# IBM/AdaMML

Hardware: AMD Instinct MI355X
Metric: clips/sec (train fwd+bwd) RGB+Audio AdaMML @224^2, 5 seg (higher is better)
Workload: dtype bf16

## Files before the change

### adamml_amd/csrc/conv_gemm.hip

```cpp
#include "common.h"
#include "tile.h"
#include "conv_internal.h"
#include "../../include/adamml_hip.h"
#include <stdlib.h>
#include <stdio.h>


namespace {

constexpr int BP = 128;
constexpr int BK = 32;

struct ConvP {
    const bf16_t* x;
    const bf16_t* w;
    const float* in_scale;
    const float* in_shift;
    bf16_t* y;
    double* stats;
    int N, H, W, Cin, OH, OW, Cout, KH, KW, stride, pad, up, up_shift, act, accumulate;
    int P, K, cin_shift, n_ptiles, n_ctiles, tpb;
    size_t gx, gy;
    int in_gstride;
    const bf16_t* bn_z;
// ... 1201 lines not shown

extern "C" int adamml_conv_fwd_bn_add_next_supported(const adamml_conv_desc_t* d, int next_cout) {
    return d && next_cout > 0 && adamml_conv_fwd_bn_add_supported(d) && adamml_conv1x1_fadd_next_supported(d, next_cout) ? 1 : 0;
}

extern "C" int adamml_conv_fwd_bn_add_next(const adamml_conv_desc_t* d, const void* x, const void* w_packed, const float* in_scale,
                                           const float* in_shift, const float* bn_vec, const void* idn, const float* id_scale,
                                           const float* id_shift, int id_gstride, int act, void* out, uint8_t* mask_out, const void* w_next,
                                           void* y_next, double* stats_next, hipStream_t stream) {
    if (!d || !x || !w_packed || !bn_vec || !out || !w_next || !y_next) return adamml_set_error(ADAMML_EINVAL, "conv_fwd_bn_add_next: null argument");
    if (!adamml_conv_fwd_bn_add_next_supported(d, 64))
        return adamml_set_error(ADAMML_EUNSUPPORTED, "conv_fwd_bn_add_next: 1x1 / stride-1, 64 -> 256 channels, next conv 256 -> 64 only");
    return adamml_conv1x1_fadd_next_launch(d, x, w_packed, in_scale, in_shift, bn_vec, idn, id_scale, id_shift, id_gstride, act, out, mask_out,
                                           w_next, y_next, stats_next, stream);
}

extern "C" int adamml_conv_fwd_bn_add_tpool_supported(const adamml_conv_desc_t* d, int frames, int act, int lazy_input) {
    if (!adamml_conv_fwd_bn_add_supported(d)) return 0;
    if (!(frames == 2 || frames == 4 || frames == 8) || d->N % frames || d->Cout % 128 || act != ADAMML_ACT_RELU) return 0;
    if (lazy_input && d->Cin > 512) return 0;
    return 1;
}

extern "C" int adamml_conv_fwd_bn_add_tpool_streams(const adamml_conv_desc_t* d, int frames) {
    if (!d) return 0;
    if (adamml_conv1x1_fadd_tpool_stream_supported(d, frames)) return 2;
    return adamml_conv1x1_fadd_tpool_supported(d, frames) ? 1 : 0;
}

extern "C" int adamml_conv_fwd_bn_add_tpool(const adamml_conv_desc_t* d, const void* x, const void* w_packed, const float* in_scale,
                                            const float* in_shift, const float* bn_vec, const void* idn, const float* id_scale,
                                            const float* id_shift, int id_gstride, int act, int frames, void* pooled, uint16_t* code,
                                            hipStream_t stream) {
    if (!adamml_conv_fwd_bn_add_tpool_supported(d, frames, act, in_scale != nullptr))
        return adamml_set_error(ADAMML_EUNSUPPORTED, "conv_fwd_bn_add_tpool: 1x1 / stride-1 conv, Cout %% 128 == 0, ReLU, 2 / 4 / 8 frames per clip");
    if (!bn_vec || !idn || !pooled) return adamml_set_error(ADAMML_EINVAL, "conv_fwd_bn_add_tpool: null argument");
    if (adamml_conv1x1_fadd_tpool_stream_supported(d, frames))
        return adamml_conv1x1_fadd_tpool_stream_launch(d, x, w_packed, in_scale, in_shift, bn_vec, idn, id_scale, id_shift, id_gstride, act, frames, pooled,
                                                       code, stream);
    if (adamml_conv1x1_fadd_tpool_supported(d, frames))
        return adamml_conv1x1_fadd_tpool_launch(d, x, w_packed, in_scale, in_shift, bn_vec, idn, id_scale, id_shift, id_gstride, act, frames, pooled, code,
                                                stream);
    FaddEpi f{bn_vec, idn, id_scale, id_shift, id_gstride, act, nullptr, frames, pooled, code};
    return conv_launch(d, x, w_packed, in_scale, in_shift, pooled, nullptr, nullptr, nullptr, 0, stream, nullptr, nullptr, nullptr, nullptr, &f);
}

static int conv_dgrad_stride2(const adamml_conv_desc_t* d, const void* dz, const void* w, void* dx, int accumulate, double* sums,
                              const void* z_in, const float* bn_vec, int act, hipStream_t stream) {
    const adamml_conv_desc_t g = dgrad_desc(d, accumulate);
    const int taps = d->KH * d->KW;
    for (int ph = 0; ph < 2; ++ph)
        for (int pw = 0; pw < 2; ++pw) {
            DgradClass c;
            c.nt = 0; c.code = 0; c.ph = ph; c.pw = pw;
            c.OHc = (d->H - ph + 1) / 2; c.OWc = (d->W - pw + 1) / 2;
            if (c.OHc <= 0 || c.OWc <= 0) continue;
            for (int kh = 0; kh < d->KH; ++kh) {
                if ((ph + d->pad - kh) & 1) continue;
                const int dh = (ph + d->pad - kh) / 2;
                for (int kw = 0; kw < d->KW; ++kw) {
                    if ((pw + d->pad - kw) & 1) continue;
                    const int dw = (pw + d->pad - kw) / 2;
                    const unsigned wt = (unsigned)(taps - 1 - (kh * d->KW + kw));
                    c.code |= ((unsigned)dh | ((unsigned)dw << 1) | (wt << 2)) << (8 * c.nt);
                    ++c.nt;
                }
            }
            if (c.nt == 0 && accumulate) continue;
            int rc = conv_launch(&g, dz, w, nullptr, nullptr, dx, sums, z_in, bn_vec, act, stream, &c);
            if (rc) return rc;
        }
    return ADAMML_OK;
}

static bool dgrad_stride2_ok(const adamml_conv_desc_t* d) {
    const bool k3 = d->KH == 3 && d->KW == 3 && d->pad == 1, k1 = d->KH == 1 && d->KW == 1 && d->pad == 0;
    return d->stride == 2 && (k3 || k1) && (d->up <= 1) && ilog2_exact(d->Cout) >= 0 &&
           d->OH == (d->H + 2 * d->pad - d->KH) / 2 + 1 && d->OW == (d->W + 2 * d->pad - d->KW) / 2 + 1;
}

extern "C" int adamml_conv_bwd_data_bn(const adamml_conv_desc_t* d, const void* dz, const void* w_dgrad_packed, void* dx,
                                       const void* z_in, const float* bn_vec, int act, double* sums, hipStream_t stream) {
    if (!d || !z_in || !bn_vec || !sums) return adamml_set_error(ADAMML_EINVAL, "conv_bwd_data_bn: null argument");
    if (dgrad_stride2_ok(d)) return conv_dgrad_stride2(d, dz, w_dgrad_packed, dx, 0, sums, z_in, bn_vec, act, stream);
    const adamml_conv_desc_t g = dgrad_desc(d, 0, true);
    return conv_launch(&g, dz, w_dgrad_packed, nullptr, nullptr, dx, sums, z_in, bn_vec, act, stream);
}

extern "C" int adamml_conv_bwd_data_dual_supported(const adamml_conv_desc_t* d) {
    return d && d->KH == 1 && d->KW == 1 && d->stride == 1 && d->pad == 0 && d->Cout <= 512 && d->Cin % 8 == 0 && d->Cout % 8 == 0 ? 1 : 0;
}

extern "C" int adamml_conv_bwd_data_dual(const adamml_conv_desc_t* d, const void* g, const void* z, const float* aff, void* dz_side,
                                         const void* w_dgrad_packed, void* dx, int accumulate, const void* z_in, const float* bn_vec,
                                         int act, double* sums, hipStream_t stream) {
    if (!d || !g || !z || !aff) return adamml_set_error(ADAMML_EINVAL, "conv_bwd_data_dual: null argument");
    if (!adamml_conv_bwd_data_dual_supported(d))
        return adamml_set_error(ADAMML_EUNSUPPORTED, "conv_bwd_data_dual: only 1x1 / stride-1 convs with Cout <= 512");
    if ((z_in != nullptr) != (bn_vec != nullptr) || (z_in != nullptr) != (sums != nullptr))
        return adamml_set_error(ADAMML_EINVAL, "conv_bwd_data_dual: incomplete BatchNorm epilogue operands");
    if (z_in && accumulate) return adamml_set_error(ADAMML_EUNSUPPORTED, "conv_bwd_data_dual: the BatchNorm epilogue does not accumulate");
    if (adamml_conv1x1_narrow_dual_supported(d))
        return adamml_conv1x1_narrow_dual_launch(d, g, z, aff, dz_side, w_dgrad_packed, dx, accumulate, z_in, bn_vec, act, sums, stream);
    const adamml_conv_desc_t gd = dgrad_desc(d, accumulate);
    DualIn di{z, aff, dz_side};
    return conv_launch(&gd, g, w_dgrad_packed, nullptr, nullptr, dx, sums, z_in, bn_vec, act, stream, nullptr, nullptr, &di);
}

extern "C" int adamml_conv_bwd_data_alg_streams(const adamml_conv_desc_t* d) {
    return d && d->KH == 1 && d->KW == 1 && d->stride == 1 && d->pad == 0 && adamml_alg_stream_supported(d->Cout, d->Cin) ? 1 : 0;
}

extern "C" int adamml_conv_bwd_data_alg(const adamml_conv_desc_t* d, const void* g, const void* a, const float* a_scale, const float* a_shift,
                                        const void* w_alg, const float* epi_add, void* dx, int accumulate, const void* z_in,
                                        const float* bn_vec, int act, double* sums, hipStream_t stream) {
    if (!d || !g || !a || !w_alg || !epi_add || !dx) return adamml_set_error(ADAMML_EINVAL, "conv_bwd_data_alg: null argument");
    if (!(d->KH == 1 && d->KW == 1 && d->stride == 1 && d->pad == 0)) return adamml_set_error(ADAMML_EUNSUPPORTED, "conv_bwd_data_alg: only 1x1 / stride-1 convs");
    if ((z_in != nullptr) != (bn_vec != nullptr) || (z_in != nullptr) != (sums != nullptr))
        return adamml_set_error(ADAMML_EINVAL, "conv_bwd_data_alg: incomplete BatchNorm epilogue operands");
    if (z_in && accumulate) return adamml_set_error(ADAMML_EUNSUPPORTED, "conv_bwd_data_alg: the BatchNorm epilogue does not accumulate");
    if (adamml_alg_stream_supported(d->Cout, d->Cin))
        return adamml_alg_stream_launch(d, g, a, a_scale, a_shift, w_alg, epi_add, dx, accumulate, z_in, bn_vec, act, sums, stream);
    adamml_conv_desc_t gd = dgrad_desc(d, accumulate);
    gd.act = d->act; gd.in_gstride = d->in_gstride;
    CatIn c{a, d->Cin, (size_t)d->Cin * (d->Cout + d->Cin), epi_add};
    return conv_launch(&gd, g, w_alg, a_scale, a_shift, dx, sums, z_in, bn_vec, act, stream, nullptr, nullptr, nullptr, &c);
}

static bool res_1x1(const adamml_conv_desc_t* d) {
    return d && d->KH == 1 && d->KW == 1 && d->stride == 1 && d->pad == 0 && d->Cin % 8 == 0 && d->Cout % 8 == 0;
}

static bool res_3x3(const adamml_conv_desc_t* d) {
    return d && d->KH == 3 && d->KW == 3 && d->stride == 1 && d->pad == 1 && d->up <= 1 && d->Cin == d->Cout && d->Cin >= 64 &&
           ilog2_exact(d->Cin) >= 0 && d->OH == d->H && d->OW == d->W;
}

extern "C" int adamml_conv_bwd_data_res_supported(const adamml_conv_desc_t* d) {
    return res_1x1(d) || res_3x3(d) ? 1 : 0;
}

static bool res_3x3_c64(const adamml_conv_desc_t* d) {
    if (!res_3x3(d)) return false;
    const adamml_conv_desc_t g = dgrad_desc(d, 0, true);
    return adamml_conv3x3_c64_res_supported(&g);
}

extern "C" int adamml_conv_bwd_data_res_streams(const adamml_conv_desc_t* d) {
    if (res_3x3_c64(d)) return 2;
    return res_1x1(d) && adamml_res_stream_supported(d) ? 1 : 0;
}

extern "C" int adamml_conv_bwd_data_res(const adamml_conv_desc_t* d, const void* dz, const void* w_dgrad_packed, void* dx,
                                        int accumulate, const void* res_out, const uint8_t* res_mask, int res_act, const void* z_a, const float* vec_a,
                                        double* sums_a, const void* z_b, const float* vec_b, double* sums_b,
                                        hipStream_t stream) {
    if (!d || !res_out || !sums_a || (z_a && !vec_a)) return adamml_set_error(ADAMML_EINVAL, "conv_bwd_data_res: null argument");
    if ((z_b != nullptr) != (vec_b != nullptr) || (z_b != nullptr) != (sums_b != nullptr))
        return adamml_set_error(ADAMML_EINVAL, "conv_bwd_data_res: incomplete second BatchNorm operand");
    if (!adamml_conv_bwd_data_res_supported(d))
        return adamml_set_error(ADAMML_EUNSUPPORTED, "conv_bwd_data_res: only 1x1 / stride-1 convs and 3x3 / pad-1 / stride-1 convs with Cin == Cout (a power of two >= 64)");
    if (accumulate && res_mask && !z_a && res_1x1(d) && adamml_res_stream_supported(d))
        return adamml_res_stream_launch(d, dz, w_dgrad_packed, dx, res_mask, sums_a, z_b, vec_b, sums_b, stream);
    const adamml_conv_desc_t g = dgrad_desc(d, accumulate, d->KH > 1);
    if (!z_b && res_3x3_c64(d))
        return adamml_conv3x3_c64_res_launch(&g, dz, w_dgrad_packed, dx, res_out, res_mask, res_act, z_a, vec_a, sums_a, stream);
    ResEpi r{res_out, res_mask, res_act, z_b, vec_b, sums_b};
    return conv_launch(&g, dz, w_dgrad_packed, nullptr, nullptr, dx, sums_a, z_a, vec_a, ACT_NONE, stream, nullptr, &r);
}
// ... 45 lines not shown
```

### adamml_amd/csrc/conv_internal.h

```cpp
#pragma once
#include "common.h"
#include "../../include/adamml_hip.h"

void launch_wgrad_reduce(const float* ws, float* dw, size_t n, int nsplit, int taps, int cin, int store, int groups, hipStream_t stream);
int adamml_launch_split_reduce(const float* ws, float* dw, size_t n, int nsplit, hipStream_t stream, int taps = 1, int cin = 1);
int adamml_launch_split_reduce_grouped(const float* ws, float* out, size_t n, int nsplit, int groups, int cin, hipStream_t stream);

bool adamml_conv3x3_c64_supported(const adamml_conv_desc_t* d);
int adamml_conv3x3_c64_launch(const adamml_conv_desc_t* d, const void* x, const void* w_packed, const float* in_scale,
                              const float* in_shift, void* y, double* stats, const void* bn_z, const float* bn_vec, int bn_act,
                              hipStream_t stream);
bool adamml_conv3x3_c64_res_supported(const adamml_conv_desc_t* d);
int adamml_conv3x3_c64_res_launch(const adamml_conv_desc_t* d, const void* dz, const void* w_dgrad_packed, void* dx, const void* res_out,
                                  const uint8_t* res_mask, int res_act, const void* z_a, const float* vec_a, double* sums_a, hipStream_t stream);
bool adamml_conv3x3_c64_wgrad_supported(const adamml_conv_desc_t* d, int cin_true);
int adamml_conv3x3_c64_wgrad_blocks(const adamml_conv_desc_t* d, int* tpb_out);
int adamml_conv3x3_c64_wgrad_launch(const adamml_conv_desc_t* d, const void* dz, const void* x, const float* in_scale,
                                    const float* in_shift, float* ws, hipStream_t stream);

bool adamml_conv1x1_narrow_fwd_supported(const adamml_conv_desc_t* d);
int adamml_conv1x1_narrow_fwd_launch(const adamml_conv_desc_t* d, const void* x, const void* w_packed, const float* in_scale, const float* in_shift,
                                     void* y, double* stats, hipStream_t stream);
bool adamml_conv1x1_narrow_wgrad_supported(const adamml_conv_desc_t* d, int cin_true);
int adamml_conv1x1_narrow_wgrad_launch(const adamml_conv_desc_t* d, const void* dz, const void* x, const float* in_scale, const float* in_shift,
                                       float* ws, int max_blocks_per_group, int* nblk_out, hipStream_t stream);
bool adamml_conv1x1_narrow_dual_supported(const adamml_conv_desc_t* d);
int adamml_conv1x1_narrow_dual_launch(const adamml_conv_desc_t* d, const void* g, const void* z, const float* aff, void* dz_side,
                                      const void* w_dgrad_packed, void* dx, int accumulate, const void* z_in, const float* bn_vec, int act,
                                      double* sums, hipStream_t stream);
bool adamml_conv1x1_narrow_dgrad_epi_supported(const adamml_conv_desc_t* d);
int adamml_conv1x1_narrow_dgrad_epi_launch(const adamml_conv_desc_t* d, const void* dz, const void* w_packed, void* dx, const void* z_in,
                                           const float* bn_vec, int act, double* sums, hipStream_t stream);

bool adamml_conv1x1_wide_expand_supported(const adamml_conv_desc_t* d);
int adamml_conv1x1_wide_expand_launch(const adamml_conv_desc_t* d, const void* x, const void* w_packed, const float* in_scale, const float* in_shift,
                                      void* y, double* stats, hipStream_t stream);

int adamml_conv1x1_fadd_stream_supported(const adamml_conv_desc_t* d);
int adamml_conv1x1_fadd_stream_launch(const adamml_conv_desc_t* d, const void* x, const void* w_packed, const float* in_scale, const float* in_shift,
                                      const float* bn_vec, const void* idn, const float* id_scale, const float* id_shift, int id_gstride, int act,
                                      void* out, uint8_t* mask_out, hipStream_t stream);
int adamml_conv1x1_fadd_tpool_stream_supported(const adamml_conv_desc_t* d, int frames);
int adamml_conv1x1_fadd_tpool_stream_launch(const adamml_conv_desc_t* d, const void* x, const void* w_packed, const float* in_scale, const float* in_shift,
                                            const float* bn_vec, const void* idn, const float* id_scale, const float* id_shift, int id_gstride, int act,
                                            int frames, void* pooled, uint16_t* code, hipStream_t stream);

bool adamml_conv1x1_fadd_next_supported(const adamml_conv_desc_t* d, int next_cout);
int adamml_conv1x1_fadd_next_launch(const adamml_conv_desc_t* d, const void* x, const void* w_packed, const float* in_scale, const float* in_shift,
                                    const float* bn_vec, const void* idn, const float* id_scale, const float* id_shift, int id_gstride, int act,
                                    void* out, uint8_t* mask_out, const void* w1_packed, void* y1, double* stats1, hipStream_t stream);
bool adamml_conv1x1_fadd_tpool_supported(const adamml_conv_desc_t* d, int frames);
int adamml_conv1x1_fadd_tpool_launch(const adamml_conv_desc_t* d, const void* x, const void* w_packed, const float* in_scale, const float* in_shift,
                                     const float* bn_vec, const void* idn, const float* id_scale, const float* id_shift, int id_gstride, int act,
                                     int frames, void* pooled, uint16_t* code, hipStream_t stream);

bool adamml_alg_stream_supported(int Cout, int Cin);
int adamml_alg_stream_launch(const adamml_conv_desc_t* d, const void* g, const void* a, const float* a_scale, const float* a_shift,
                             const void* w_alg, const float* epi_add, void* dx, int accumulate, const void* z_in, const float* bn_vec,
                             int act, double* sums, hipStream_t stream);

int adamml_res_stream_supported(const adamml_conv_desc_t* d);
int adamml_res_stream_launch(const adamml_conv_desc_t* d, const void* dz, const void* w_dgrad_packed, void* dx, const uint8_t* res_mask, double* sums_a,
                             const void* z_b, const float* vec_b, double* sums_b, hipStream_t stream);
int adamml_res_prod_stream_supported(const adamml_conv_desc_t* d, int a_channels);
size_t adamml_res_prod_stream_workspace(const adamml_conv_desc_t* d);
int adamml_res_prod_stream_launch(const adamml_conv_desc_t* d, const void* dz, const void* w_dgrad_packed, void* dx, const uint8_t* res_mask,
                                  double* sums_a, const void* a, const float* a_scale, const float* a_shift, int a_act, int a_gstride,
                                  float* prod, void* workspace, size_t workspace_bytes, hipStream_t stream);
```

### adamml_amd/hip.py

```python
import ctypes
import os
from ctypes import c_void_p, c_int, c_int32, c_int64, c_float, c_double, c_size_t, c_char_p, POINTER, Structure, byref

import torch

_HERE = os.path.dirname(os.path.abspath(__file__))
LIB_PATH = os.environ.get("ADAMML_HIP_LIB") or os.path.join(_HERE, "libadamml_hip.so")

ACT_NONE, ACT_RELU, ACT_RELU6 = 0, 1, 2
STAT_SLOTS = 32


class ConvDesc(Structure):
    _fields_ = [(n, c_int32) for n in ("N", "H", "W", "Cin", "OH", "OW", "Cout", "KH", "KW", "stride", "pad", "up", "act",
                                      "accumulate", "groups", "in_gstride")]

    def __init__(self, *args, **kw):
        super().__init__(*args, **kw)
        if self.groups < 1:
            self.groups = 1


_P, _I, _F, _D, _Z, _L = c_void_p, c_int, c_float, c_double, c_size_t, c_int64
_DESC = POINTER(ConvDesc)
# ... 40 lines not shown
    "adamml_bn_eval_affine": [_P, _P, _P, _P, _F, _P, _P, _I, _P],
    "adamml_bn_act_add": [_P, _P, _P, _I, _I, _P, _P, _P, _I, _P, _Z, _I, _I, _P],
    "adamml_act_bwd_from_output": [_P, _P, _I, _P, _Z, _P],
    "adamml_bn_bwd_reduce": [_P, _P, _P, _I, _P, _Z, _I, _I, _P],
    "adamml_bn_bwd_finalize": [_P, _I, _I, _D, _P, _P, _P, _P, _P, _I, _F, _P],
    "adamml_bn_bwd_finalize_affine": [_P, _I, _I, _D, _P, _P, _P, _P, _P, _P, _I, _F, _P],
    "adamml_bn_bwd_apply": [_P, _P, _P, _I, _P, _P, _Z, _I, _I, _P],
    "adamml_maxpool2d_fwd": [_P, _P, _P, _I, _I, _P, _P, _P, _I, _I, _I, _I, _I, _I, _I, _P],
    "adamml_maxpool2d_bwd": [_P, _P, _P, _I, _I, _I, _I, _I, _I, _I, _P],
    "adamml_maxpool2d_bwd_bn_reduce": [_P, _P, _P, _P, _I, _P, _I, _I, _I, _I, _I, _I, _I, _P],
    "adamml_maxpool2d_bwd_bn_apply": [_P, _P, _P, _P, _I, _P, _P, _I, _I, _I, _I, _I, _I, _I, _P],
    "adamml_temporal_pool_fwd": [_P, _P, _P, _I, _I, _P, _I, _I, _Z, _I, _I, _I, _P],
    "adamml_temporal_pool_bwd": [_P, _P, _P, _P, _I, _I, _P, _I, _I, _Z, _I, _I, _I, _P],
    "adamml_temporal_pool_bwd_res": [_P, _P, _I, _P, _P, _P, _P, _I, _I, _I, _I, _I, _P],
    "adamml_gap_fwd": [_P, _P, _P, _I, _I, _P, _I, _I, _I, _I, _P],
    "adamml_gap_bwd": [_P, _P, _I, _I, _I, _P],
    "adamml_head_fwd": [_P, _P, _P, _I, _I, _P, _F, _P, _P, _P, _P, _I, _I, _I, _I, _I, _I, _P],
    "adamml_head_bwd": [_P, _P, _F, _P, _P, _P, _I, _I, _I, _I, _I, _P],
    "adamml_colsum_f32": [_P, _P, _I, _I, _I, _P],
    "adamml_clip_to_nhwc": [_P, _P, _I, _I, _I, _I, _I, _I, _I, _I, _I, _I, _P],
    "adamml_clip_u8_to_nhwc": [_P, _P, _I, _I, _I, _I, _I, _I, _I, _I, _I, _I, _P, _P, _I, _I, _P],
    "adamml_clip_u8_rgbdiff_to_nhwc": [_P, _P, _I, _I, _I, _I, _I, _I, _I, _I, _I, _I, _P, _P, _I, _P],
    "adamml_log_spectrogram": [_P, _P, _P, _I, _I, _I, _I, _I, _F, _P],
    "adamml_video_resample_u8": [_P, _L, _P, _I, _P, _I, _I, _I, _I, _I, _I, _P],
    "adamml_jpeg_decode_u8": [_P, _L, _P, _I, _P, _L, _P, _P, _L, _I, _P],
    "adamml_gemm_f32": [_P, _L, _L, _P, _L, _L, _P, _L, _L, _P, _I, _I, _I, _I, _I, _P],
    "adamml_sgd_step": [_P, _P, _P, _Z, _F, _F, _F, _I, _I, _P],
    "adamml_adam_step": [_P, _P, _P, _P, _Z, _F, _F, _F, _F, _F, _I, _P],
    "adamml_policy_head_fwd": [_P, _P, _I, _P, _P, _P, _P, _P, _F, _P, _P, _P, _P, _P, _P, _P, _I, _I, _I, _I, _P],
    "adamml_policy_head_bwd": [_P, _P, _P, _I, _P, _P, _F, _P, _P, _P, _P, _P, _I, _I, _I, _I, _P],
    "adamml_gumbel_gate_fwd": [_P, _P, _F, _P, _P, _I, _P],
    "adamml_gumbel_gate_bwd": [_P, _P, _F, _P, _I, _P],
    "adamml_fusion_fwd": [_P, _P, _P, _P, _I, _I, _I, _I, _P],
    "adamml_fusion_bwd": [_P, _P, _P, _P, _P, _P, _P, _I, _I, _I, _I, _P],
}

_lib = None


def load():
    global _lib
    if _lib is not None:
        return _lib
    if not os.path.exists(LIB_PATH):
        raise RuntimeError("adamml_amd: %s not found -- build it with `python -c 'import __graft_entry__ as g; g.build()'`; "
                           "there is no CPU fallback for the HIP hot path" % LIB_PATH)
    lib = ctypes.CDLL(LIB_PATH)
    for name, argt in SIGNATURES.items():
        fn = getattr(lib, name)
        fn.argtypes = argt
        fn.restype = c_int
    lib.adamml_conv_bwd_weight_workspace.argtypes = [_DESC, _I]
    lib.adamml_conv_bwd_weight_workspace.restype = c_size_t
    lib.adamml_conv_stem_bwd_weight_workspace.argtypes = [_DESC]
    lib.adamml_conv_stem_bwd_weight_workspace.restype = c_size_t
    lib.adamml_dwconv_bwd_weight_workspace.argtypes = [_DESC]
    lib.adamml_dwconv_bwd_weight_workspace.restype = c_size_t
    lib.adamml_conv_stem1_bwd_weight_workspace.argtypes = [_DESC]
    lib.adamml_conv_stem1_bwd_weight_workspace.restype = c_size_t
    lib.adamml_conv_stem1_supported.argtypes = [_DESC]
    lib.adamml_conv_stem1_supported.restype = c_int
    lib.adamml_gram_colsum_workspace.argtypes = [_Z, _I, _I]
    lib.adamml_gram_colsum_workspace.restype = c_size_t
    lib.adamml_gram_colsum_supported.argtypes = [_I]
    lib.adamml_gram_colsum_supported.restype = c_int
    lib.adamml_conv_bwd_data_res_prod_workspace.argtypes = [_DESC]
    lib.adamml_conv_bwd_data_res_prod_workspace.restype = c_size_t
    lib.adamml_conv_bwd_data_res_prod_supported.argtypes = [_DESC, _I]
    lib.adamml_conv_bwd_data_res_prod_supported.restype = c_int
    lib.adamml_conv_bwd_data_res_prod_streams.argtypes = [_DESC, _I]
    lib.adamml_conv_bwd_data_res_prod_streams.restype = c_int
    lib.adamml_conv_fwd_bn_add_streams.argtypes = [_DESC]
    lib.adamml_conv_fwd_bn_add_streams.restype = c_int
    lib.adamml_conv_bwd_data_res_streams.argtypes = [_DESC]
    lib.adamml_conv_bwd_data_res_streams.restype = c_int
    lib.adamml_conv_fwd_bn_add_tpool_streams.argtypes = [_DESC, _I]
    lib.adamml_conv_fwd_bn_add_tpool_streams.restype = c_int
    lib.adamml_gemm_f32_uses_mfma.argtypes = [_P, _L, _L, _P, _L, _L, _I]
    lib.adamml_gemm_f32_uses_mfma.restype = c_int
    lib.adamml_clip_to_nhwc_four_pixel.argtypes = [_P, _P, _I, _I, _I, _I, _I]
    lib.adamml_clip_to_nhwc_four_pixel.restype = c_int
    lib.adamml_conv_bwd_data_alg_streams.argtypes = [_DESC]
    lib.adamml_conv_bwd_data_alg_streams.restype = c_int
    lib.adamml_conv_fused_input_supported.argtypes = [_DESC]
    lib.adamml_conv_fused_input_supported.restype = c_int
    lib.adamml_conv1x1_narrow_supported.argtypes = [_DESC, c_int]
    lib.adamml_conv1x1_narrow_supported.restype = c_int
    lib.adamml_conv1x1_wide_supported.argtypes = [_DESC, c_int]
    lib.adamml_conv1x1_wide_supported.restype = c_int
    lib.adamml_conv_fwd_bn_add_supported.argtypes = [_DESC]
    lib.adamml_conv_fwd_bn_add_supported.restype = c_int
    lib.adamml_conv_fwd_bn_add_next_supported.argtypes = [_DESC, c_int]
    lib.adamml_conv_fwd_bn_add_next_supported.restype = c_int
    lib.adamml_conv_fwd_bn_add_tpool_supported.argtypes = [_DESC, _I, _I, _I]
    lib.adamml_conv_fwd_bn_add_tpool_supported.restype = c_int
    lib.adamml_conv_bwd_data_dual_supported.argtypes = [_DESC]
    lib.adamml_conv_bwd_data_dual_supported.restype = c_int
    lib.adamml_conv_bwd_data_res_supported.argtypes = [_DESC]
    lib.adamml_conv_bwd_data_res_supported.restype = c_int
    lib.adamml_temporal_pool_bwd_res_supported.argtypes = [_I, _I, _I]
    lib.adamml_temporal_pool_bwd_res_supported.restype = c_int
    lib.adamml_dwconv_bwd_data_bn_supported.argtypes = [_DESC]
    lib.adamml_dwconv_bwd_data_bn_supported.restype = c_int
    lib.adamml_temporal_pool_bwd_code_prod_supported.argtypes = [c_int, c_int, c_int]
    lib.adamml_temporal_pool_bwd_code_prod_supported.restype = c_int
    lib.adamml_temporal_pool_bwd_code_prod_workspace.argtypes = [c_int, c_int, c_int, c_int, c_int, c_int]
    lib.adamml_temporal_pool_bwd_code_prod_workspace.restype = c_size_t
    lib.adamml_dwconv_bwd_fused_supported.argtypes = [_DESC]
    lib.adamml_dwconv_bwd_fused_supported.restype = c_int
    lib.adamml_dwconv_bwd_fused_workspace.argtypes = [_DESC]
    lib.adamml_dwconv_bwd_fused_workspace.restype = c_size_t
    lib.adamml_jpeg_decode_workspace.argtypes = [_L]
    lib.adamml_jpeg_decode_workspace.restype = c_size_t
    lib.adamml_jpeg_decode_parallel_supported.argtypes = [_I, _I, _I, _I, _I, _L]
    lib.adamml_jpeg_decode_parallel_supported.restype = c_int
    lib.adamml_conv_stem_supported.argtypes = [_DESC]
    lib.adamml_conv_stem_supported.restype = c_int
    lib.adamml_plan_run.argtypes = [c_void_p, c_int, c_void_p, c_int, c_void_p, c_int, c_void_p, c_int]
    lib.adamml_plan_run.restype = c_int
    lib.adamml_plan_events_create.argtypes = [c_void_p, c_int]
    lib.adamml_plan_events_create.restype = c_int
    lib.adamml_plan_events_destroy.argtypes = [c_void_p, c_int]
    lib.adamml_plan_events_destroy.restype = c_int
    lib.adamml_plan_num_entry_points.restype = c_int
    lib.adamml_pack_block_elems.restype = c_int
    lib.adamml_version.restype = c_int
    lib.adamml_last_error_string.restype = c_char_p
    lib.adamml_set_deterministic.argtypes = [_I]
    lib.adamml_set_deterministic.restype = c_int
    lib.adamml_get_deterministic.restype = c_int
    _lib = lib
    return lib


def set_deterministic(on=True):
    lib = _lib if _lib is not None else load()
    rc = lib.adamml_set_deterministic(1 if on else 0)
    if rc != 0:
        raise RuntimeError("adamml_set_deterministic failed (%d): %s" % (rc, lib.adamml_last_error_string().decode()))


def deterministic():
    return bool((_lib if _lib is not None else load()).adamml_get_deterministic())


_raw_stream = getattr(torch._C, "_cuda_getCurrentRawStream", None)


def _stream():
    if _raw_stream is not None:
        return _raw_stream(torch.cuda.current_device())
    return torch.cuda.current_stream().cuda_stream


recorder = None


def ptr(t):
    if t is None:
        return None
    if recorder is not None:
        recorder.keep.append(t)
    return t.data_ptr()


class LaunchProfiler:
# ... 80 lines not shown
```

### include/adamml_hip.h

```cpp
#ifndef ADAMML_HIP_H
#define ADAMML_HIP_H
#include <stddef.h>
#include <stdint.h>
#ifdef __cplusplus
extern "C" {
#endif

typedef struct ihipStream_t* hipStream_t;
typedef struct ihipEvent_t* hipEvent_t;

#define ADAMML_API __attribute__((visibility("default")))

#define ADAMML_STAT_SLOTS 32

#define ADAMML_ACT_NONE 0
#define ADAMML_ACT_RELU 1
#define ADAMML_ACT_RELU6 2

typedef struct {
    int32_t N, H, W, Cin;
    int32_t OH, OW, Cout;
    int32_t KH, KW, stride, pad;
    int32_t up;
    int32_t act;
    int32_t accumulate;
    int32_t groups;
    int32_t in_gstride;
} adamml_conv_desc_t;

ADAMML_API int adamml_version(void);
ADAMML_API const char* adamml_last_error_string(void);
ADAMML_API int adamml_set_deterministic(int on);
ADAMML_API int adamml_get_deterministic(void);

ADAMML_API int adamml_conv_fwd(const adamml_conv_desc_t* d, const void* x, const void* w_packed, const float* in_scale,
                    const float* in_shift, void* y, double* stats, hipStream_t stream);
ADAMML_API int adamml_conv_fused_input_supported(const adamml_conv_desc_t* d);
ADAMML_API int adamml_conv1x1_narrow_supported(const adamml_conv_desc_t* d, int kind);
ADAMML_API int adamml_conv1x1_wide_supported(const adamml_conv_desc_t* d, int kind);
ADAMML_API int adamml_conv_fwd_bn_add_supported(const adamml_conv_desc_t* d);
ADAMML_API int adamml_conv_fwd_bn_add_streams(const adamml_conv_desc_t* d);
ADAMML_API int adamml_conv_fwd_bn_add(const adamml_conv_desc_t* d, const void* x, const void* w_packed, const float* in_scale, const float* in_shift,
                           const float* bn_vec, const void* idn, const float* id_scale, const float* id_shift, int id_gstride, int act,
                           void* out, uint8_t* mask_out, hipStream_t stream);
ADAMML_API int adamml_conv_fwd_bn_add_next_supported(const adamml_conv_desc_t* d, int next_cout);
ADAMML_API int adamml_conv_fwd_bn_add_next(const adamml_conv_desc_t* d, const void* x, const void* w_packed, const float* in_scale, const float* in_shift,
                                const float* bn_vec, const void* idn, const float* id_scale, const float* id_shift, int id_gstride, int act,
                                void* out, uint8_t* mask_out, const void* w_next, void* y_next, double* stats_next, hipStream_t stream);
ADAMML_API int adamml_conv_fwd_bn_add_tpool_supported(const adamml_conv_desc_t* d, int frames, int act, int lazy_input);
ADAMML_API int adamml_conv_fwd_bn_add_tpool_streams(const adamml_conv_desc_t* d, int frames);
ADAMML_API int adamml_conv_fwd_bn_add_tpool(const adamml_conv_desc_t* d, const void* x, const void* w_packed, const float* in_scale, const float* in_shift,
                                 const float* bn_vec, const void* idn, const float* id_scale, const float* id_shift, int id_gstride, int act,
                                 int frames, void* pooled, uint16_t* code, hipStream_t stream);
ADAMML_API int adamml_gram_stats(const void* w_packed, const float* G, const float* s, double* sums, int Cout, int Cin, int groups, hipStream_t stream);
ADAMML_API int adamml_gram_colsum_supported(int C);
ADAMML_API size_t adamml_gram_colsum_workspace(size_t P, int C, int groups);
ADAMML_API int adamml_gram_colsum(const void* x, const float* scale, const float* shift, int gstride, int act, float* G, float* s, size_t P, int C,
                       int groups, void* workspace, size_t workspace_bytes, hipStream_t stream);
ADAMML_API int adamml_conv_bwd_data(const adamml_conv_desc_t* d, const void* dz, const void* w_dgrad_packed, void* dx,
                         int accumulate, hipStream_t stream);
ADAMML_API int adamml_conv_bwd_data_bn(const adamml_conv_desc_t* d, const void* dz, const void* w_dgrad_packed, void* dx, const void* z_in,
                            const float* bn_vec, int act, double* sums, hipStream_t stream);

ADAMML_API int adamml_conv_bwd_data_dual_supported(const adamml_conv_desc_t* d);
ADAMML_API int adamml_bn_bwd_affine(const float* coef, const float* vec, float* aff, int C, int groups, hipStream_t stream);
ADAMML_API int adamml_conv_bwd_data_dual(const adamml_conv_desc_t* d, const void* g, const void* z, const float* aff, void* dz_side,
                              const void* w_dgrad_packed, void* dx, int accumulate, const void* z_in, const float* bn_vec, int act,
                              double* sums, hipStream_t stream);

ADAMML_API int adamml_conv_bwd_weight_grouped(const adamml_conv_desc_t* d, const void* dz, const float* dz_scale, const float* dz_shift, int dz_act,
                                   int dz_gstride, const void* x, const float* in_scale, const float* in_shift, float* out, int cin_true,
                                   void* workspace, size_t workspace_bytes, hipStream_t stream);
ADAMML_API int adamml_lazy_colsum(const void* x, const float* scale, const float* shift, int gstride, int act, float* s, size_t P, int C, int groups,
                       hipStream_t stream);
ADAMML_API int adamml_alg_sumfix(const float* w, const float* P, const float* vec, double* sums, int Cout, int Cin, int groups, hipStream_t stream);
ADAMML_API int adamml_alg_pack(const float* w, const float* aff, const float* m_pre, void* w_alg, float* epi_add, int Cout, int Cin, int groups,
                    hipStream_t stream);
ADAMML_API int adamml_alg_wgrad_combine(const float* w, const float* aff, const float* P, const float* G, const float* wg_pre, const float* s, float* dw,
                             int Cout, int Cin, int groups, hipStream_t stream);
ADAMML_API int adamml_conv_bwd_data_alg_streams(const adamml_conv_desc_t* d);
ADAMML_API int adamml_conv_bwd_data_alg(const adamml_conv_desc_t* d, const void* g, const void* a, const float* a_scale, const float* a_shift,
                             const void* w_alg, const float* epi_add, void* dx, int accumulate, const void* z_in, const float* bn_vec,
                             int act, double* sums, hipStream_t stream);

ADAMML_API int adamml_conv_bwd_data_res_supported(const adamml_conv_desc_t* d);
ADAMML_API int adamml_conv_bwd_data_res_streams(const adamml_conv_desc_t* d);
ADAMML_API int adamml_conv_bwd_data_res(const adamml_conv_desc_t* d, const void* dz, const void* w_dgrad_packed, void* dx,
                             int accumulate, const void* res_out, const uint8_t* res_mask, int res_act, const void* z_a, const float* vec_a,
                             double* sums_a, const void* z_b, const float* vec_b, double* sums_b, hipStream_t stream);

ADAMML_API int adamml_conv_bwd_data_res_prod_supported(const adamml_conv_desc_t* d, int a_channels);
ADAMML_API size_t adamml_conv_bwd_data_res_prod_workspace(const adamml_conv_desc_t* d);
ADAMML_API int adamml_conv_bwd_data_res_prod_streams(const adamml_conv_desc_t* d, int a_channels);
ADAMML_API int adamml_conv_bwd_data_res_prod(const adamml_conv_desc_t* d, const void* dz, const void* w_dgrad_packed, void* dx, const uint8_t* res_mask,
                                  int res_act, double* sums_a, const void* a, const float* a_scale, const float* a_shift, int a_act,
                                  int a_gstride, int a_channels, float* prod, void* workspace, size_t workspace_bytes, hipStream_t stream);

ADAMML_API size_t adamml_conv_bwd_weight_workspace(const adamml_conv_desc_t* d, int cin_true);
ADAMML_API int adamml_conv_bwd_weight(const adamml_conv_desc_t* d, const void* dz, const void* x, const float* in_scale,
                           const float* in_shift, float* dw, int cin_true, void* workspace, size_t workspace_bytes,
                           hipStream_t stream);
ADAMML_API int adamml_pack_conv_weight(const float* w, void* out, int cout, int cin_true, int cin_pad, int kh, int kw, int mode,
                            hipStream_t stream);

ADAMML_API int adamml_conv_stem_supported(const adamml_conv_desc_t* d);
ADAMML_API int adamml_pack_stem_weight(const float* w, void* out, int cout, int cin_true, hipStream_t stream);
ADAMML_API int adamml_conv_stem_fwd(const adamml_conv_desc_t* d, const void* x, const void* w_stem_packed, void* y, double* stats,
                         hipStream_t stream);
ADAMML_API size_t adamml_conv_stem_bwd_weight_workspace(const adamml_conv_desc_t* d);
ADAMML_API int adamml_conv_stem_bwd_weight(const adamml_conv_desc_t* d, const void* dz, const void* x, float* dw, int cin_true,
                                void* workspace, size_t workspace_bytes, hipStream_t stream);

ADAMML_API int adamml_dwconv_fwd(const adamml_conv_desc_t* d, const void* x, const float* w_tapmajor, const float* in_scale,
                      const float* in_shift, void* y, double* stats, hipStream_t stream);
ADAMML_API int adamml_dwconv_bwd_data(const adamml_conv_desc_t* d, const void* dz, const float* w_tapmajor, void* dx,
                           int accumulate, hipStream_t stream);
ADAMML_API int adamml_dwconv_bwd_data_bn_supported(const adamml_conv_desc_t* d);
ADAMML_API int adamml_dwconv_bwd_data_bn(const adamml_conv_desc_t* d, const void* dz, const float* w_tapmajor, void* dx, const void* z_in,
                              const float* bn_vec, int act, double* sums, hipStream_t stream);
ADAMML_API size_t adamml_dwconv_bwd_weight_workspace(const adamml_conv_desc_t* d);
ADAMML_API int adamml_dwconv_bwd_fused_supported(const adamml_conv_desc_t* d);
ADAMML_API size_t adamml_dwconv_bwd_fused_workspace(const adamml_conv_desc_t* d);
ADAMML_API int adamml_dwconv_bwd_fused(const adamml_conv_desc_t* d, const void* g, const void* z, const float* aff, const float* w_tapmajor,
                            const void* x, const float* x_vec, int x_act, void* dx, double* sums, float* dw, void* workspace,
                            size_t workspace_bytes, hipStream_t stream);
ADAMML_API int adamml_conv_stem1_supported(const adamml_conv_desc_t* d);
ADAMML_API int adamml_conv_stem1_fwd(const adamml_conv_desc_t* d, const float* x, size_t image_stride, size_t group_stride, const float* w_tapmajor,
                          void* y, double* stats, hipStream_t stream);
ADAMML_API size_t adamml_conv_stem1_bwd_weight_workspace(const adamml_conv_desc_t* d);
ADAMML_API int adamml_conv_stem1_bwd_weight(const adamml_conv_desc_t* d, const void* dz, const float* x, size_t image_stride, size_t group_stride,
                                 float* dw , void* workspace,
                                 size_t workspace_bytes, hipStream_t stream);
ADAMML_API int adamml_dwconv_bwd_weight(const adamml_conv_desc_t* d, const void* dz, const void* x, const float* in_scale,
                             const float* in_shift, float* dw, void* workspace, size_t workspace_bytes, hipStream_t stream);

ADAMML_API int adamml_stats_collapse(const double* stats, double* out, int C, int groups, hipStream_t stream);
ADAMML_API int adamml_bn_finalize(const double* stats, int nslots, int groups, double count, const float* gamma, const float* beta,
                       float* running_mean, float* running_var, float momentum, float eps, float* bn_vec, int C,
                       hipStream_t stream);
ADAMML_API int adamml_bn_eval_affine(const float* gamma, const float* beta, const float* running_mean, const float* running_var,
                          float eps, float* scale, float* shift, int C, hipStream_t stream);
ADAMML_API int adamml_bn_act_add(const void* z, const float* scale, const float* shift, int z_gstride, int act, const void* idn,
                      const float* id_scale, const float* id_shift, int id_gstride, void* out, size_t P, int C, int groups,
                      hipStream_t stream);
ADAMML_API int adamml_bn_act_add_mask(const void* z, const float* scale, const float* shift, int z_gstride, int act, const void* idn,
// ... 122 lines not shown
```

Before: 3438.

## Add fused quad-phase stride-2 3x3 dgrad kernel with BatchNorm backward epilogue

Adds a dedicated kernel for stride-2 3x3 data-gradient convolution that splits the output into its four parity phases. Each block loads one dz patch into LDS once and reuses it across all phase tap sets, while weight slabs are streamed through a per-wave ring buffer. The kernel fuses the BatchNorm/activation backward epilogue and the stat reduction. It is enabled by default only for Cout==128 layers with enough workgroups, trading extra LDS and code complexity for less redundant dz loading than the generic stride-2 dgrad path.

```diff
diff --git a/adamml_amd/csrc/conv_dgrad_s2.hip b/adamml_amd/csrc/conv_dgrad_s2.hip
--- /dev/null
+++ b/adamml_amd/csrc/conv_dgrad_s2.hip
@@ -0,0 +1,288 @@
+#include "common.h"
+#include "tile.h"
+#include "conv_internal.h"
+#include "../../include/adamml_hip.h"
+#include <stdlib.h>
+
+namespace {
+
+constexpr int QT = 256;
+constexpr int QBC = 64;
+constexpr int QPIX = 64;
+constexpr int QROWS = 88;
+constexpr int QKS_BYTES = QROWS * 64;
+constexpr int QNB = 8;
+constexpr int QRING_BYTES = QNB * 1024 * (QT / 64);
+constexpr int QCROW = QBC * 2 + 16;
+constexpr int QNRE = 8;
+constexpr int QCPR = QBC / 8;
+constexpr int QTAB = 9 * 16 + QNB;
+constexpr int QEPI_BYTES = 4 * QPIX * QCROW;
+
+struct QuadP {
+    const bf16_t* dz;
+    const bf16_t* w;
+    bf16_t* dx;
+    const bf16_t* z;
+    const float* bn_vec;
+    double* stats;
+    int N, Hz, Wz, C, Co, bn_act, nth, ntw, n_tiles, n_ctiles, tpb, nks, tab_off;
+    size_t gz, gx;
+};
+
+struct QuadRound { int nt, view, cls[4], wt[4]; };
+constexpr QuadRound QROUND[4] = {{1, 3, {3, 0, 0, 0}, {8, 0, 0, 0}},
+                                 {2, 2, {3, 2, 0, 0}, {6, 7, 0, 0}},
+                                 {2, 1, {3, 1, 0, 0}, {2, 5, 0, 0}},
+                                 {4, 0, {0, 1, 2, 3}, {4, 3, 1, 0}}};
+constexpr unsigned long long QWT_PACK = 0x8ull | (0x76ull << 16) | (0x52ull << 32) | (0x0134ull << 48);
+constexpr bool quad_pack_matches_rounds() {
+    for (int r = 0; r < 4; ++r)
+        for (int t = 0; t < QROUND[r].nt; ++t)
+            if ((int)((QWT_PACK >> (16 * r + 4 * t)) & 0xfull) != QROUND[r].wt[t]) return false;
+    return true;
+}
+static_assert(quad_pack_matches_rounds(), "QWT_PACK is QROUND's tap list");
+
+__device__ __forceinline__ int quad_lds_off(int row, int chunk) {
+    return row * 64 + ((chunk ^ (((row >> 3) & 1) << 1)) << 4);
+}
+
+template <int TW>
+__global__ __launch_bounds__(QT, 2) void conv_dgrad_s2_quad_kernel(QuadP p) {
+    constexpr int TH = QPIX / TW, PW = TW + 1, PPIX = (TH + 1) * PW, XW = 2 * TW;
+    static_assert(PPIX <= QROWS, "patch image");
+    extern __shared__ __attribute__((aligned(1024))) char smem[];
+    {
+        const int g = blockIdx.y;
+        p.dz += (size_t)g * p.gz;
+        p.dx += (size_t)g * p.gx;
+        p.z += (size_t)g * p.gx;
+        p.bn_vec += (size_t)g * 4 * p.Co;
+        p.stats += (size_t)g * ADAMML_STAT_SLOTS * 2 * p.Co;
+    }
+    const int tid = threadIdx.x, lane = tid & 63, wave = tid >> 6, li = lane & 15, lg = lane >> 4;
+    const int bid = (int)xcd_contiguous(blockIdx.x, gridDim.x);
+    const int ctile = bid % p.n_ctiles, pgrp = bid / p.n_ctiles;
+    const int c0 = ctile * QBC;
+    const int C = p.C, nks = p.nks, oH = 2 * p.Hz, oW = 2 * p.Wz;
+    const int patch_bytes = nks * QKS_BYTES;
+    const unsigned lds0 = (unsigned)(size_t)(__attribute__((address_space(3))) char*)smem;
+    const bf16_t* zeros = reinterpret_cast<const bf16_t*>(g_zero_page);
+
+    int boff[4][4];
+#pragma unroll
+    for (int v = 0; v < 4; ++v)
+#pragma unroll
+        for (int pt = 0; pt < 4; ++pt) {
+            const int q = pt * 16 + li;
+            boff[v][pt] = quad_lds_off((q / TW + (v >> 1)) * PW + (q % TW) + (v & 1), lg);
+        }
+    const char* ring = smem + patch_bytes + wave * (QNB * 1024);
+    const unsigned ring0 = lds0 + patch_bytes + wave * (QNB * 1024);
+    const int aoff = quad_lds_off(li, lg);
+    const bf16_t* wsrc;
+    {
+        const int row = lane >> 2, ch = (lane & 3) ^ (((row >> 3) & 1) << 1);
+        wsrc = p.w + (size_t)(c0 + wave * 16 + row) * (9 * C) + ch * 8;
+    }
+    const int ns = 9 * nks;
+    int* s_tab = reinterpret_cast<int*>(smem + p.tab_off);
+    for (int j = tid; j < ns + QNB; j += QT) {
+        const int jc = j < ns ? j : ns - 1;
+        int r, rem, sh;
+        if (jc < nks) { r = 0; rem = jc; sh = 0; }
+        else if (jc < 3 * nks) { r = 1; rem = jc - nks; sh = 1; }
+        else if (jc < 5 * nks) { r = 2; rem = jc - 3 * nks; sh = 1; }
+        else { r = 3; rem = jc - 5 * nks; sh = 2; }
+        const int ks = rem >> sh, t = rem & ((1 << sh) - 1);
+        s_tab[j] = (int)((QWT_PACK >> (16 * r + 4 * t)) & 0xfull) * C + ks * 32;
+    }
+    __syncthreads();
+    auto issue_slab = [&](int j, int off) {
+        glds16(wsrc + off, __builtin_amdgcn_readfirstlane(ring0 + (unsigned)(j & (QNB - 1)) * 1024u));
+    };
+
+    const int ech = tid & (QCPR - 1), erow0 = tid / QCPR;
+    const int eco = c0 + ech * 8;
+    f32x8 esum, esq, cadd;
+#pragma unroll
+    for (int i = 0; i < 8; ++i) esum[i] = esq[i] = cadd[i] = 0.f;
+
+    for (int it = 0; it < p.tpb; ++it) {
+        const int tile = pgrp * p.tpb + it;
+        if (tile >= p.n_tiles) break;
+        const int n = tile / (p.nth * p.ntw), trem = tile - n * (p.nth * p.ntw);
+        const int h0 = (trem / p.ntw) * TH, w0 = (trem % p.ntw) * TW;
+
+        for (int e0 = wave * 64; e0 < nks * (QROWS * 4); e0 += QT) {
+            const int e = e0 + lane;
+            const int ks = e / (QROWS * 4), rem = e - ks * (QROWS * 4);
+            const int row = rem >> 2, ch = (rem & 3) ^ (((row >> 3) & 1) << 1);
+            const int pr = row / PW, pc = row - pr * PW;
+            const int h = h0 + pr, w = w0 + pc;
+            const bool ok = row < PPIX && h < p.Hz && w < p.Wz;
+            const bf16_t* src = ok ? p.dz + ((size_t)(n * p.Hz + h) * p.Wz + w) * C + ks * 32 + ch * 8 : zeros;
+            glds16(src, __builtin_amdgcn_readfirstlane(lds0 + (unsigned)e0 * 16u));
+        }
+#pragma unroll
+        for (int j = 0; j < QNB; ++j) issue_slab(j, s_tab[j]);
+        const bool full = h0 + TH <= p.Hz && w0 + TW <= p.Wz;
+        bf16x8 zr[QNRE];
+        unsigned zoff[QNRE], okbits = 0;
+#pragma unroll
+        for (int j = 0; j < QNRE; ++j) {
+            const int er = erow0 + j * 32;
+            const int rr = er / XW, cc = er % XW;
+            const bool ok = rr < 2 * (p.Hz - h0) && cc < 2 * (p.Wz - w0);
+            okbits |= ok ? 1u << j : 0u;
+            const int oh = 2 * h0 + (ok ? rr : 0), ow = 2 * w0 + (ok ? cc : 0);
+            zoff[j] = ((unsigned)(n * oH + oh) * (unsigned)oW + (unsigned)ow) * (unsigned)p.Co + (unsigned)eco;
+            zr[j] = *reinterpret_cast<const bf16x8*>(p.z + zoff[j]);
+        }
+        asm volatile("s_waitcnt vmcnt(%0)" ::"n"(QNB + QNRE) : "memory");
+        __syncthreads();
+
+        f32x4 acc[4][4];
+#pragma unroll
+        for (int c = 0; c < 4; ++c)
+#pragma unroll
+            for (int pt = 0; pt < 4; ++pt) acc[c][pt] = f32x4{0.f, 0.f, 0.f, 0.f};
+
+        int j0 = 0;
+        static_for<4>([&](auto rc) {
+            constexpr QuadRound R = QROUND[decltype(rc)::value];
+            for (int ks = 0; ks < nks; ++ks) {
+                if (j0 + R.nt - 1 < QNB) asm volatile("s_waitcnt vmcnt(%0)" ::"n"(QNB - R.nt + QNRE) : "memory");
+                else asm volatile("s_waitcnt vmcnt(%0)" ::"n"(QNB - R.nt) : "memory");
+                bf16x8 fa[R.nt], fb[4];
+                int noff[R.nt];
+#pragma unroll
+                for (int t = 0; t < R.nt; ++t) {
+                    fa[t] = *reinterpret_cast<const bf16x8*>(ring + ((j0 + t) & (QNB - 1)) * 1024 + aoff);
+                    noff[t] = s_tab[j0 + QNB + t];
+                }
+#pragma unroll
+                for (int pt = 0; pt < 4; ++pt)
+                    fb[pt] = *reinterpret_cast<const bf16x8*>(smem + ks * QKS_BYTES + boff[R.view][pt]);
+                asm volatile("s_waitcnt lgkmcnt(0)" ::: "memory");
+#pragma unroll
+                for (int t = 0; t < R.nt; ++t) issue_slab(j0 + QNB + t, noff[t]);
+#pragma unroll
+                for (int t = 0; t < R.nt; ++t)
+#pragma unroll
+                    for (int pt = 0; pt < 4; ++pt)
+                        acc[R.cls[t]][pt] = __builtin_amdgcn_mfma_f32_16x16x32_bf16(fa[t], fb[pt], acc[R.cls[t]][pt], 0, 0, 0);
+                j0 += R.nt;
+            }
+        });
+        asm volatile("s_waitcnt vmcnt(0)" ::: "memory");
+        const f32x8 sc = load_f32x8(p.bn_vec + eco), sh = load_f32x8(p.bn_vec + p.Co + eco);
+        const f32x8 mu = load_f32x8(p.bn_vec + 2 * p.Co + eco), is = load_f32x8(p.bn_vec + 3 * p.Co + eco);
+        __syncthreads();
+
+#pragma unroll
+        for (int c = 0; c < 4; ++c)
+#pragma unroll
+            for (int pt = 0; pt < 4; ++pt) {
+                const int q = pt * 16 + li;
+                const int er = (2 * (q / TW) + (c >> 1)) * XW + 2 * (q % TW) + (c & 1);
+                *reinterpret_cast<bf16x4*>(smem + er * QCROW + (wave * 16 + lg * 4) * 2) = f32_to_bf4(acc[c][pt]);
+            }
+        __syncthreads();
+        auto epilogue = [&](auto full_c) {
+            constexpr bool FULL = decltype(full_c)::value;
+#pragma unroll
+            for (int j = 0; j < QNRE; ++j) {
+                if (FULL || ((okbits >> j) & 1u)) {
+                    const int er = erow0 + j * 32;
+                    f32x8 f = bf8_to_f32(*reinterpret_cast<const bf16x8*>(smem + er * QCROW + ech * 16)) + cadd;
+                    const f32x8 zv = bf8_to_f32(zr[j]);
+#pragma unroll
+                    for (int i = 0; i < 8; ++i) f[i] *= act_mask(fmaf(zv[i], sc[i], sh[i]), p.bn_act);
+                    const bf16x8 v = f32_to_bf8(f);
+                    *reinterpret_cast<bf16x8*>(p.dx + zoff[j]) = v;
+                    f = bf8_to_f32(v);
+                    esum += f;
+#pragma unroll
+                    for (int i = 0; i < 8; ++i) esq[i] += f[i] * (zv[i] - mu[i]) * is[i];
+                }
+            }
+        };
+        if (full) epilogue(std::true_type{}); else epilogue(std::false_type{});
+        __syncthreads();
+    }
+
+    float* red = reinterpret_cast<float*>(smem);
+#pragma unroll
+    for (int i = 0; i < 8; ++i) {
+        red[(erow0 * QCPR + ech) * 16 + i] = esum[i];
+        red[(erow0 * QCPR + ech) * 16 + 8 + i] = esq[i];
+    }
+    __syncthreads();
+    if (tid < 2 * QBC) {
+        const int which = tid / QBC, c = tid & (QBC - 1);
+        float v = red[(c >> 3) * 16 + which * 8 + (c & 7)];
+        for (int k = 1; k < 32; ++k) v += red[(k * QCPR + (c >> 3)) * 16 + which * 8 + (c & 7)];
+        stat_publish(p.stats + (which ? (size_t)p.Co : 0) + c0 + c, 2 * (size_t)p.Co, 0u, v);
+    }
+}
+
+template <int TW>
+int quad_launch_(const QuadP& p, int groups, size_t lds, hipStream_t stream) {
+    static AdamLdsOnce attr_once;
+    const int attr_dev = adamml_current_device();
+    if (!attr_once.test(attr_dev)) {
+        hipError_t e = hipFuncSetAttribute(reinterpret_cast<const void*>(conv_dgrad_s2_quad_kernel<TW>), hipFuncAttributeMaxDynamicSharedMemorySize,
+                                           QKS_BYTES * 16 + QRING_BYTES + QTAB * 4);
+        if (e != hipSuccess) return adamml_set_error(ADAMML_ELAUNCH, "conv_bwd_data_bn (quad): cannot raise the dynamic LDS limit: %s", hipGetErrorString(e));
+        attr_once.set(attr_dev);
+    }
+    const dim3 grid(ceil_div(p.n_tiles, p.tpb) * p.n_ctiles, groups);
+    hipLaunchKernelGGL((conv_dgrad_s2_quad_kernel<TW>), grid, dim3(QT), lds, stream, p);
+    return adamml_check_launch("conv_bwd_data_bn (quad)");
+}
+
+bool quad_runs(const adamml_conv_desc_t* d) {
+    if (!d || d->KH != 3 || d->KW != 3 || d->pad != 1 || d->stride != 2 || d->up > 1) return false;
+    if (d->H < 2 || d->W < 2 || (d->H & 1) || (d->W & 1) || d->OH != d->H / 2 || d->OW != d->W / 2) return false;
+    if (ilog2_exact(d->Cout) < 0 || d->Cout < 64 || d->Cout > 512) return false;
+    if (ilog2_exact(d->Cin) < 0 || d->Cin < QBC) return false;
+    return (long)d->N * d->H * d->W * d->Cin < (1L << 31);
+}
+
+}
+
+bool adamml_conv_dgrad_s2_quad_supported(const adamml_conv_desc_t* d) {
+    const char* e = getenv("ADAMML_DGRAD_S2_QUAD");
+    const int mode = e ? atoi(e) : 1;
+    if (mode == 0 || !quad_runs(d)) return false;
+    if (mode == 2) return true;
+    const long wgs = (long)d->N * ceil_div(d->OH, 4) * ceil_div(d->OW, 16) * (d->Cin / QBC) * (d->groups < 1 ? 1 : d->groups);
+    return d->Cout == 128 && d->OW >= 16 && wgs >= 4096;
+}
+
+int adamml_conv_dgrad_s2_quad_launch(const adamml_conv_desc_t* d, const void* dz, const void* w_dgrad_packed, void* dx, const void* z_in,
+                                     const float* bn_vec, int act, double* sums, hipStream_t stream) {
+    if (!quad_runs(d)) return adamml_set_error(ADAMML_EUNSUPPORTED, "conv_bwd_data_bn (quad): unsupported shape");
+    if (!dz || !w_dgrad_packed || !dx || !z_in || !bn_vec || !sums) return adamml_set_error(ADAMML_EINVAL, "conv_bwd_data_bn (quad): null argument");
+    if (d->N <= 0) return ADAMML_OK;
+    QuadP p;
+    p.dz = (const bf16_t*)dz; p.w = (const bf16_t*)w_dgrad_packed; p.dx = (bf16_t*)dx; p.z = (const bf16_t*)z_in; p.bn_vec = bn_vec; p.stats = sums;
+    p.N = d->N; p.Hz = d->OH; p.Wz = d->OW; p.C = d->Cout; p.Co = d->Cin; p.bn_act = act;
+    const int groups = d->groups < 1 ? 1 : d->groups;
+    const int TW = p.Wz <= 8 ? 8 : 16, TH = QPIX / TW;
+    p.nth = ceil_div(p.Hz, TH); p.ntw = ceil_div(p.Wz, TW);
+    p.n_tiles = p.N * p.nth * p.ntw;
+    p.n_ctiles = p.Co / QBC;
+    p.nks = p.C / 32;
+    p.gz = (size_t)d->N * p.Hz * p.Wz * p.C;
+    p.gx = (size_t)d->N * d->H * d->W * p.Co;
+    p.tpb = (int)((long)p.n_tiles * p.n_ctiles * groups / 2048);
+    if (p.tpb < 1) p.tpb = 1;
+    if (p.tpb > 8) p.tpb = 8;
+    const size_t opnd = (size_t)p.nks * QKS_BYTES + QRING_BYTES;
+    p.tab_off = (int)(opnd > (size_t)QEPI_BYTES ? opnd : (size_t)QEPI_BYTES);
+    const size_t lds = (size_t)p.tab_off + QTAB * 4;
+    return TW == 8 ? quad_launch_<8>(p, groups, lds, stream) : quad_launch_<16>(p, groups, lds, stream);
+}
diff --git a/adamml_amd/csrc/conv_gemm.hip b/adamml_amd/csrc/conv_gemm.hip
--- a/adamml_amd/csrc/conv_gemm.hip
+++ b/adamml_amd/csrc/conv_gemm.hip
@@ -1307,9 +1307,15 @@
 extern "C" int adamml_conv_bwd_data_bn(const adamml_conv_desc_t* d, const void* dz, const void* w_dgrad_packed, void* dx,
                                        const void* z_in, const float* bn_vec, int act, double* sums, hipStream_t stream) {
     if (!d || !z_in || !bn_vec || !sums) return adamml_set_error(ADAMML_EINVAL, "conv_bwd_data_bn: null argument");
+    if (dgrad_stride2_ok(d) && adamml_conv_dgrad_s2_quad_supported(d))
+        return adamml_conv_dgrad_s2_quad_launch(d, dz, w_dgrad_packed, dx, z_in, bn_vec, act, sums, stream);
     if (dgrad_stride2_ok(d)) return conv_dgrad_stride2(d, dz, w_dgrad_packed, dx, 0, sums, z_in, bn_vec, act, stream);
     const adamml_conv_desc_t g = dgrad_desc(d, 0, true);
     return conv_launch(&g, dz, w_dgrad_packed, nullptr, nullptr, dx, sums, z_in, bn_vec, act, stream);
+}
+
+extern "C" int adamml_conv_bwd_data_bn_quad_streams(const adamml_conv_desc_t* d) {
+    return d && dgrad_stride2_ok(d) && adamml_conv_dgrad_s2_quad_supported(d) ? 1 : 0;
 }
 
 extern "C" int adamml_conv_bwd_data_dual_supported(const adamml_conv_desc_t* d) {
diff --git a/adamml_amd/csrc/conv_internal.h b/adamml_amd/csrc/conv_internal.h
--- a/adamml_amd/csrc/conv_internal.h
+++ b/adamml_amd/csrc/conv_internal.h
@@ -17,6 +17,10 @@
 int adamml_conv3x3_c64_wgrad_blocks(const adamml_conv_desc_t* d, int* tpb_out);
 int adamml_conv3x3_c64_wgrad_launch(const adamml_conv_desc_t* d, const void* dz, const void* x, const float* in_scale,
                                     const float* in_shift, float* ws, hipStream_t stream);
+
+bool adamml_conv_dgrad_s2_quad_supported(const adamml_conv_desc_t* d);
+int adamml_conv_dgrad_s2_quad_launch(const adamml_conv_desc_t* d, const void* dz, const void* w_dgrad_packed, void* dx, const void* z_in,
+                                     const float* bn_vec, int act, double* sums, hipStream_t stream);
 
 bool adamml_conv1x1_narrow_fwd_supported(const adamml_conv_desc_t* d);
 int adamml_conv1x1_narrow_fwd_launch(const adamml_conv_desc_t* d, const void* x, const void* w_packed, const float* in_scale, const float* in_shift,
diff --git a/adamml_amd/hip.py b/adamml_amd/hip.py
--- a/adamml_amd/hip.py
+++ b/adamml_amd/hip.py
@@ -146,6 +146,8 @@
     lib.adamml_clip_to_nhwc_four_pixel.restype = c_int
     lib.adamml_conv_bwd_data_alg_streams.argtypes = [_DESC]
     lib.adamml_conv_bwd_data_alg_streams.restype = c_int
+    lib.adamml_conv_bwd_data_bn_quad_streams.argtypes = [_DESC]
+    lib.adamml_conv_bwd_data_bn_quad_streams.restype = c_int
     lib.adamml_conv_fused_input_supported.argtypes = [_DESC]
     lib.adamml_conv_fused_input_supported.restype = c_int
     lib.adamml_conv1x1_narrow_supported.argtypes = [_DESC, c_int]
diff --git a/include/adamml_hip.h b/include/adamml_hip.h
--- a/include/adamml_hip.h
+++ b/include/adamml_hip.h
@@ -61,6 +61,7 @@
                          int accumulate, hipStream_t stream);
 ADAMML_API int adamml_conv_bwd_data_bn(const adamml_conv_desc_t* d, const void* dz, const void* w_dgrad_packed, void* dx, const void* z_in,
                             const float* bn_vec, int act, double* sums, hipStream_t stream);
+ADAMML_API int adamml_conv_bwd_data_bn_quad_streams(const adamml_conv_desc_t* d);
 
 ADAMML_API int adamml_conv_bwd_data_dual_supported(const adamml_conv_desc_t* d);
 ADAMML_API int adamml_bn_bwd_affine(const float* coef, const float* vec, float* aff, int C, int groups, hipStream_t stream);
```

Result: no change. 3444 (median of 2 runs) (+0.2%).
